# sevagh/demucs.cpp

Measured on AMD Instinct MI355X. Metric: audio-sec/s (xRT) htdemucs-4s 44.1kHz stereo, ~4-min track with overlap-add (BASELINE configs[2]), higher is better.
Workload: dtype f32 (exact bf16x3 operand split, fp32 accumulate)

## Files before the change

### demucs_cpp_amd/csrc/api.cpp

```cpp
#include "api_internal.h"
#include "tracks_plan.h"

#include <algorithm>
#include <atomic>
#include <cstdarg>
#include <cstdio>
#include <cstdlib>
#include <cmath>
#include <cstring>
#include <cctype>
#include <cerrno>
#include <climits>
#include <fcntl.h>
#include <pthread.h>
#include <signal.h>
#include <sys/mman.h>
#include <sys/stat.h>
#include <unistd.h>

using namespace dmx;

static thread_local std::string g_err;
int dmx_fail(int code, const char *fmt, ...)
{
// ... 2157 lines not shown
        rc = fail(DMX_ERR_HIP, "%s: hipMalloc failed", fn);
    if (rc == DMX_OK && (hipMemcpy(dIn, planes, inBytes, hipMemcpyHostToDevice) != hipSuccess ||
                         (mix && hipMemcpy(dMix, mix, mixBytes, hipMemcpyHostToDevice) != hipSuccess)))
        rc = fail(DMX_ERR_HIP, "%s: upload failed", fn);
    if (rc == DMX_OK)
        rc = dmx_remix_encode_device(device, dIn, n_sources, n, n, dMix, spec, dOut, dPeaks, nullptr);
    if (rc == DMX_OK && hipDeviceSynchronize() != hipSuccess)
        rc = fail(DMX_ERR_HIP, "%s: the kernels failed: %s", fn, hipGetErrorString(hipGetLastError()));
    for (int o = 0; rc == DMX_OK && o < nOut; ++o)
        if (hipMemcpy((unsigned char *)out + (size_t)(o * bytes), dOut + (size_t)(o * devStride), (size_t)bytes, hipMemcpyDeviceToHost) != hipSuccess)
            rc = fail(DMX_ERR_HIP, "%s: download failed", fn);
    if (rc == DMX_OK && peaks && hipMemcpy(peaks, dPeaks, sizeof(float) * (size_t)nOut, hipMemcpyDeviceToHost) != hipSuccess)
        rc = fail(DMX_ERR_HIP, "%s: download failed", fn);
    for (void *p : {(void *)dIn, (void *)dOut, (void *)dPeaks, (void *)dMix})
        if (p)
            (void)hipFree(p);
    return rc;
}

extern "C" int64_t dmx_flac_bound(int bits, int64_t n) { return flac_bound(bits, n); }
extern "C" int64_t dmx_flac_workspace_bytes(int bits, int64_t n) { return flac_workspace_bytes(bits, n); }

static int flac_check(const char *fn, int bits, int64_t n, int sample_rate)
{
    if (bits != 16 && bits != 24)
        return fail(DMX_ERR_ARG, "%s: bits %d (16 or 24)", fn, bits);
    if (n < 1 || n >= (int64_t)1 << 36)
        return fail(DMX_ERR_ARG, "%s: n = %lld, must be in [1, 2^36)", fn, (long long)n);
    if (sample_rate < 1 || sample_rate > 655350)
        return fail(DMX_ERR_ARG, "%s: sample_rate %d not in [1, 655350]", fn, sample_rate);
    return DMX_OK;
}

extern "C" int dmx_flac_encode_device(int device, const void *d_pcm, int bits, int64_t n, int sample_rate, void *d_out, int64_t *d_size,
                                      void *d_work, void *stream)
{
    const char *fn = "dmx_flac_encode_device";
    DMXCHK(flac_check(fn, bits, n, sample_rate));
    if (!d_pcm || !d_out || !d_size || !d_work)
        return fail(DMX_ERR_ARG, "%s: null %s pointer", fn, !d_pcm ? "d_pcm" : !d_out ? "d_out" : !d_size ? "d_size" : "d_work");
    if (((uintptr_t)d_pcm & 15) != 0 || ((uintptr_t)d_work & 15) != 0 || ((uintptr_t)d_size & 7) != 0)
        return fail(DMX_ERR_ARG, "%s: d_pcm and d_work must be 16-byte aligned, d_size 8-byte aligned", fn);
    HIPCHK(hipSetDevice(device));
    launch_flac_encode((const unsigned char *)d_pcm, 0, bits, n, sample_rate, 1, (unsigned char *)d_out, 0, (long long *)d_size,
                       (unsigned char *)d_work, (hipStream_t)stream);
    HIPCHK(hipGetLastError());
    return DMX_OK;
}

extern "C" int dmx_flac_encode(int device, const void *pcm, int bits, int64_t n, int sample_rate, void *out, int64_t *size)
{
    const char *fn = "dmx_flac_encode";
    DMXCHK(flac_check(fn, bits, n, sample_rate));
    if (!pcm || !out || !size)
        return fail(DMX_ERR_ARG, "%s: null %s pointer", fn, !pcm ? "pcm" : !out ? "out" : "size");
    HIPCHK(hipSetDevice(device));
    const size_t inBytes = (size_t)n * 2 * (size_t)(bits / 8);
    const i64 bound = flac_bound(bits, n), workBytes = flac_workspace_bytes(bits, n);
    unsigned char *dIn = nullptr, *dOut = nullptr, *dWork = nullptr;
    int64_t *dSize = nullptr;
    int64_t got = 0;
    int rc = DMX_OK;
    if (hipMalloc((void **)&dIn, DMX_OUTPUT_STRIDE(inBytes)) != hipSuccess || hipMalloc((void **)&dOut, (size_t)bound) != hipSuccess ||
        hipMalloc((void **)&dWork, (size_t)workBytes) != hipSuccess || hipMalloc((void **)&dSize, sizeof(int64_t)) != hipSuccess)
        rc = fail(DMX_ERR_HIP, "%s: hipMalloc failed", fn);
    if (rc == DMX_OK && hipMemcpy(dIn, pcm, inBytes, hipMemcpyHostToDevice) != hipSuccess)
        rc = fail(DMX_ERR_HIP, "%s: upload failed", fn);
    if (rc == DMX_OK)
        rc = dmx_flac_encode_device(device, dIn, bits, n, sample_rate, dOut, dSize, dWork, nullptr);
    if (rc == DMX_OK && hipDeviceSynchronize() != hipSuccess)
        rc = fail(DMX_ERR_HIP, "%s: the kernels failed: %s", fn, hipGetErrorString(hipGetLastError()));
    if (rc == DMX_OK && hipMemcpy(&got, dSize, sizeof(int64_t), hipMemcpyDeviceToHost) != hipSuccess)
        rc = fail(DMX_ERR_HIP, "%s: download failed", fn);
    if (rc == DMX_OK && (got < 42 || got > bound))
        rc = fail(DMX_ERR_HIP, "%s: internal error (%lld encoded bytes, bound %lld)", fn, (long long)got, (long long)bound);
    if (rc == DMX_OK && hipMemcpy(out, dOut, (size_t)got, hipMemcpyDeviceToHost) != hipSuccess)
        rc = fail(DMX_ERR_HIP, "%s: download failed", fn);
    for (void *p : {(void *)dIn, (void *)dOut, (void *)dWork, (void *)dSize})
        if (p)
            (void)hipFree(p);
    if (rc == DMX_OK)
        *size = got;
    return rc;
}

extern "C" int dmx_tracks_infer_flac(dmx_ctx *c, const dmx_model *const *models, int n_models, const float *weights, int n_tracks,
                                     const float *const *audio, const int64_t *n, int n_shifts, float overlap, const int *shift_offsets,
                                     const dmx_remix_spec *spec, int sample_rate, void *const *out, int64_t *sizes, float *peaks, int layout,
                                     dmx_progress_fn progress, void *user)
{
    TracksCall a = remix_call("dmx_tracks_infer_flac", c, models, n_models, weights, spec);
    a.kind = TRACKS_OUT_FLAC, a.flacRate = sample_rate, a.flacSizes = sizes;
    a.n_tracks = n_tracks, a.audio = audio, a.n = n, a.n_shifts = n_shifts, a.overlap = overlap, a.shift_offsets = shift_offsets;
    a.out = out, a.peaks = peaks, a.layout = layout, a.progress = progress, a.user = user;
    return tracks_call(a);
}

extern "C" int dmx_debug_tap(dmx_ctx *c, const char *name, int64_t *shape, float *host_dst)
{
    if (!c || !name || !shape || c->lastBatch < 1)
        return -1;
    (void)hipSetDevice(c->m->device);
    Plan *p = get_plan(c, c->lastBatch);
    for (const Op &op : p->ops)
        if (op.kind == OP_TAP && op.name == name)
        {
            int nd = 0;
            i64 per = 1;
            shape[nd++] = p->B;
            for (int j = 0; j < 4 && op.tap.shape[j] > 0; ++j)
            {
                shape[nd++] = op.tap.shape[j];
                per *= op.tap.shape[j];
            }
            if (host_dst)
            {
                (void)hipStreamSynchronize(c->stream);
                for (int b = 0; b < p->B; ++b)
                    if (hipMemcpy(host_dst + b * per, c->dA + op.tap.off + b * op.tap.batchStride, sizeof(float) * (size_t)per,
                                  hipMemcpyDeviceToHost) != hipSuccess)
                        return -1;
            }
            return nd;
        }
    return -1;
}

extern "C" int dmx_debug_n_ops(const dmx_ctx *c)
{
    if (!c)
        return 0;
    auto it = c->plans.find(c->maxBatch);
    return it == c->plans.end() ? 0 : (int)it->second->ops.size();
}

static void op_work(const Op &op, const char *&kernel, double &flops, double &bytes)
{
    static const char *cfgNames[] = {"igemm_128x128", "igemm_64x64", "igemm_128x96", "igemm_128x48", "igemm_256x16", "igemm_128x32",
                                     "igemm_128x64",  "igemm_64x128", "dgemm_direct", "igemm_64x64", "igemm_64x96", "igemm_64x48",
                                     "igemm_64x32",   "igemm_64x64",  "igemm_128x16", "igemm_32x128", "igemm_32x64", "igemm_256x128", "igemm_256x128w4", "igemm_lin256x128", "igemm_256x96"};
    static_assert(sizeof(cfgNames) / sizeof(cfgNames[0]) == kNumTileCfgs, "one label per tile configuration");
    flops = bytes = 0;
    kernel = "?";
    switch (op.kind)
    {
    case OP_IGEMM:
    {
        const IGemm &g = op.g;
        const double M = (double)g.B * g.P1 * g.P0;
        kernel = cfgNames[g.cfg];
        if (g.split)
        {
            static const char *splitNames[kNumTileCfgs] = {"igemm_split_128x128", nullptr, "igemm_split_128x96", "igemm_split_128x48", nullptr, "igemm_split_128x32d", "igemm_split_128x64d",
                                                            "igemm_split_64x128", nullptr, "igemm_split_64x64", "igemm_split_64x96", "igemm_split_64x48",
                                                            "igemm_split_128x32d", "igemm_split_128x64d", nullptr, "igemm_split_32x128", "igemm_split_32x64", nullptr, nullptr,
                                                            nullptr, nullptr};
            if (splitNames[g.cfg])
                kernel = splitNames[g.cfg];
            if (g.split == 2)
                kernel = g.cfg == 0 ? "igemm_splith_128x128" : g.cfg == 7 ? "igemm_splith_64x128" : kernel;
            else if (g.cfg == 0 || g.cfg == 2)
            {
                GemmArgs k{};
                fill_gemm_geometry(k, g);
                k.rowstat = g.rowstat >= 0 ? reinterpret_cast<float *>(1) : nullptr;
                const int wide = igemm_split_is_wide(g.cfg, k);
                if (wide)
                    kernel = wide == 256 ? "igemm_split_128x256" : wide == 192 ? "igemm_split_128x192" : "igemm_split_128x96d";
            }
        }
        flops = 2.0 * M * g.N * g.K;
        double in = (double)g.B * g.L1 * g.L0 * g.Cin, w = (double)g.N * g.K, out = 0;
        if (g.epi == EPI_LINEAR || g.epi == EPI_SCALE_RES)
            out = M * g.N;
        else if (g.epi == EPI_KPL || g.epi == EPI_VT)
            out = M * g.N;
        else if (g.epi == EPI_GLU || g.epi == EPI_GN_GLU_SCALE_RES)
            out = M * g.N / 2;
        else if (g.epi == EPI_TRCONV)
            out = (double)g.B * g.P1 * g.Lout * g.Cout;
        double res = g.res >= 0 ? out : 0;
        bytes = 4.0 * (in + w + out + res);
        break;
    }
    case OP_ATTENTION:
    {
        const Attention &t = op.at;
        kernel = t.split ? "attention_split" : "attention";
        flops = 4.0 * t.B * t.H * (double)t.Tq * t.Tk * t.hs;
        bytes = 4.0 * t.B * t.H * t.hs * (2.0 * t.Tq + 2.0 * t.Tk);
        break;
    }
    case OP_DCONV_ROW:
    {
        const DconvRow &r = op.dr;
        const double M = (double)r.B * r.T * r.F, hp = (r.hid + 3) / 4 * 4;
        kernel = "dconv_row";
        flops = 2.0 * (2.0 * M * hp * 3.0 * r.C + 2.0 * M * (hp + 2) * hp + 2.0 * M * 2.0 * r.C * hp);
        bytes = 4.0 * 2.0 * M * r.C;
        break;
    }
    case OP_STATS_REDUCE:
        kernel = "stats_reduce";
        bytes = 8.0 * op.sr.B * op.sr.R * op.sr.NB;
        break;
    case OP_STFT:
        kernel = "stft";
        flops = (double)op.stft.B * op.stft.T * 5.0 * 4096 * 12;
        bytes = 4.0 * op.stft.B * ((double)op.stft.seg * 2 + (double)op.stft.T * 2048 * 4);
        break;
    case OP_LAYERNORM:
        kernel = "layernorm";
        bytes = 8.0 * op.ln.rows * op.ln.D;
        break;
    case OP_GN_APPLY:
        kernel = "gn_apply";
        bytes = 8.0 * op.gn.B * op.gn.rows * op.gn.C;
        break;
    case OP_ISTFT:
        kernel = "istft";
        if (op.istft.fused)
            break;
        flops = (double)op.istft.B * op.istft.T * op.istft.S * 5.0 * 4096 * 12;
        bytes = 4.0 * op.istft.B * op.istft.T * op.istft.S * (2048.0 * 4 + 2 * 4096.0);
        break;
    case OP_OLA:
        kernel = "ola";
        bytes = 4.0 * op.ola.B * op.ola.S * 2 * ((double)op.ola.T * 4096 + 2.0 * op.ola.seg);
        if (op.ola.x >= 0)
        {
            kernel = "istft_ola";
            flops = (double)op.ola.B * op.ola.T * op.ola.S * 5.0 * 4096 * 12;
            bytes = 4.0 * op.ola.B * ((double)op.ola.T * 2048 * 4 * op.ola.S + 4.0 * op.ola.seg * op.ola.S);
        }
        break;
    case OP_GROUP_STATS:
        kernel = "group_stats";
        bytes = 4.0 * op.gs.B * op.gs.rows * op.gs.C;
        break;
    case OP_GN_ACT:
    {
        const GnAct &g = op.ga;
        const double Co = g.mode == 2 ? g.C / 2 : g.C;
        kernel = "gn_act";
        bytes = 4.0 * g.B * ((double)g.rowsOut * g.C + (double)g.rowsOut * Co * (g.res >= 0 ? 2 : 1));
        break;
    }
    case OP_LSTM:
    {
        const Lstm &l = op.lstm;
        kernel = "lstm";
        flops = 2.0 * l.B * l.T * 2.0 * 4.0 * l.H * l.H;
        bytes = 4.0 * (l.B * (double)l.T * 10.0 * l.H + 8.0 * l.H * l.H);
        break;
    }
    case OP_LOCAL_ATTN:
    {
        const LocalAttn &l = op.la;
        kernel = "local_attn";
        flops = 4.0 * l.B * (double)l.T * l.T * l.H;
        bytes = 4.0 * l.B * l.T * ((double)l.ld + l.H);
        break;
    }
    default:
        break;
    }
}

extern "C" int dmx_debug_profile(dmx_ctx *c, int batch, int reps, char *report, int report_cap)
{
    if (!c || batch < 1 || batch > c->maxBatch || reps < 1)
        return -1;
    (void)hipSetDevice(c->m->device);
    Plan *p = get_plan(c, batch);
    hipEvent_t e0, e1;
    if (hipEventCreate(&e0) != hipSuccess || hipEventCreate(&e1) != hipSuccess)
        return -1;
    int n = 0;
    std::string all;
    char line[512];
    for (const Op &op : p->ops)
    {
        if (op.kind == OP_TAP)
            continue;
        launch_op(c, op, c->stream, p->zeroOff);
        (void)hipEventRecord(e0, c->stream);
        for (int r = 0; r < reps; ++r)
            launch_op(c, op, c->stream, p->zeroOff);
        (void)hipEventRecord(e1, c->stream);
        (void)hipEventSynchronize(e1);
        float t = 0.f;
        (void)hipEventElapsedTime(&t, e0, e1);
        const char *kernel;
        double fl, by;
        op_work(op, kernel, fl, by);
        char geom[160] = "";
        if (op.kind == OP_IGEMM)
        {
            const IGemm &g = op.g;
            const i64 M = (i64)g.B * g.P1 * g.P0;
            const i64 tiles = ((M + kTileCfgs[g.cfg].BM - 1) / kTileCfgs[g.cfg].BM) * g.NB;
            snprintf(geom, sizeof(geom), "M=%lld N=%d K=%d tiles=%lld pro=%d epi=%d lin=%d stat=%d s%d", (long long)M, g.N, g.K, (long long)tiles,
                     g.pro, g.epi, (int)(g.S1 == 1 && g.pad0 == 0 && g.seg0 == g.K), (int)(g.rowstat >= 0), op.stream);
        }
        else
            snprintf(geom, sizeof(geom), "s%d", op.stream);
        snprintf(line, sizeof(line), "%s\t%s\t%.6f\t%.6e\t%.6e\t%s\n", op.name.c_str(), kernel, t / reps, fl, by, geom);
        all += line;
        ++n;
    }
    (void)hipEventDestroy(e0);
    (void)hipEventDestroy(e1);
    if (report && report_cap > 0)
    {
        size_t k = std::min((size_t)report_cap - 1, all.size());
        std::memcpy(report, all.data(), k);
        report[k] = 0;
    }
    return n;
}
```

### demucs_cpp_amd/csrc/dgemm.hip

```cpp
#include "kernels.h"
#include <cstdlib>

namespace dmx
{

typedef float f32x4 __attribute__((ext_vector_type(4)));

__device__ __forceinline__ float dgelu(float v) { return dmx_gelu(v); }
__device__ __forceinline__ float dsigmoid(float v) { return __builtin_amdgcn_rcpf(1.0f + __expf(-v)); }
__device__ __forceinline__ unsigned fdiv(unsigned n, const FastDiv f)
{
    return f.magic ? (__umulhi(n, f.magic) >> f.shift) : (n >> f.shift);
}
__device__ __forceinline__ float4 ld4z(const float *ptr, bool ok, const float *zero)
{
    const f32x4 v = *reinterpret_cast<const f32x4 *>(ok ? ptr : zero);
    return make_float4(v[0], v[1], v[2], v[3]);
}
__device__ __forceinline__ float f4get(const float4 &v, int c) { return c == 0 ? v.x : (c == 1 ? v.y : (c == 2 ? v.z : v.w)); }

template <int NF, int S1, int SEG0, int PRO, int EPI, int PIPE>
__global__ __launch_bounds__(256) void dgemm_kernel(const GemmArgs pa, const FastDiv dP0, const FastDiv dP1)
{
    GemmArgs p = pa;
    if (gridDim.y > 1)
    {
        const int n0 = (int)blockIdx.y * pa.N;
        p.Wt += (i64)n0 * pa.Kp, p.bias += n0, p.epiW += n0, p.epiB += n0, p.scale += n0 / 2;
        p.Y += n0 / 2, p.res += n0 / 2;
    }
    constexpr int NV4 = SEG0 / 16;
    constexpr int RPL = (SEG0 % 16) / 4;
    constexpr int NV4A = NV4 > 0 ? NV4 : 1;
    constexpr int RPLA = RPL > 0 ? RPL : 1;
    const int lane = threadIdx.x & 63, l15 = lane & 15, h = lane >> 4;
    const int gwave = blockIdx.x * 4 + (threadIdx.x >> 6), nwaves = gridDim.x * 4;
    const int rowLen = p.L0 * p.Cin;

    float4 Bv[NF][S1][NV4A];
    float Br[NF][S1][RPLA];
#pragma unroll
    for (int fj = 0; fj < NF; ++fj)
    {
        const int n = fj * 16 + l15;
        const float *w = p.Wt + (i64)(n < p.Np ? n : 0) * p.Kp;
        const bool nOk = n < p.Np;
#pragma unroll
        for (int s = 0; s < S1; ++s)
        {
#pragma unroll
            for (int j = 0; j < NV4; ++j)
                Bv[fj][s][j] = ld4z(w + s * SEG0 + 16 * j + 4 * h, nOk, p.zero);
#pragma unroll
            for (int c = 0; c < RPL; ++c)
                Br[fj][s][c] = nOk ? w[s * SEG0 + 16 * NV4 + RPL * h + c] : 0.f;
        }
    }
    float4 gW4[NV4A], gB4[NV4A];
    float gWr[RPLA], gBr[RPLA];
    if (PRO == PRO_GN_GELU)
    {
#pragma unroll
        for (int j = 0; j < NV4; ++j)
        {
            gW4[j] = *reinterpret_cast<const float4 *>(p.proW + 16 * j + 4 * h);
            gB4[j] = *reinterpret_cast<const float4 *>(p.proB + 16 * j + 4 * h);
        }
#pragma unroll
        for (int c = 0; c < RPL; ++c)
        {
            gWr[c] = p.proW[16 * NV4 + RPL * h + c];
            gBr[c] = p.proB[16 * NV4 + RPL * h + c];
        }
    }
    constexpr bool CST_LDS = EPI == EPI_GN_GLU_SCALE_RES;
    __shared__ float4 cst[CST_LDS ? 4 : 1][NF][4];
    float4 biasv[CST_LDS ? 1 : NF];
    int trR[NF], trC[NF];
    if (CST_LDS)
    {
        for (int i = threadIdx.x; i < NF * 4; i += 256)
        {
            const int fj = i >> 2, hh = i & 3, n = fj * 16 + 4 * hh;
            const bool ok = n < p.N;
            cst[0][fj][hh] = ld4z(p.bias + n, ok, p.zero);
            cst[CST_LDS ? 1 : 0][fj][hh] = ld4z(p.epiW + n, ok, p.zero);
            cst[CST_LDS ? 2 : 0][fj][hh] = ld4z(p.epiB + n, ok, p.zero);
            cst[CST_LDS ? 3 : 0][fj][hh] = ld4z(p.scale + (fj >> 1) * 16 + 4 * hh, ok && (fj & 1) == 0, p.zero);
        }
        __syncthreads();
    }
#pragma unroll
    for (int fj = 0; fj < NF; ++fj)
    {
        const int n = fj * 16 + 4 * h;
        if (!CST_LDS)
            biasv[fj] = ld4z(p.bias + n, n < p.N, p.zero);
        trR[fj] = trC[fj] = 0;
        if (EPI == EPI_TRCONV)
        {
            trR[fj] = n / p.Cout;
            trC[fj] = n - trR[fj] * p.Cout;
        }
    }

    constexpr int NRES = (EPI == EPI_GLU || EPI == EPI_GN_GLU_SCALE_RES) ? (NF + 1) / 2 : 1;
    struct Stage
    {
        unsigned m, b;
        int p0, p1;
        bool rowOk;
        float aMean, aScale, eMean, eSc;
        f32x4 a4[S1][NV4A];
        float ar[S1][RPLA];
        unsigned ok4, okr;
        f32x4 resv[NRES];
    };
    const int nfrag = (int)((p.M + 15) >> 4);
    const int C2 = p.N >> 1;
    auto fetch = [&](int frag, Stage &st) {
        const unsigned m = (unsigned)frag * 16u + (unsigned)l15;
        const bool rowOk = frag < nfrag && (i64)m < p.M;
        const unsigned mm = rowOk ? m : 0u;
        const unsigned t1 = fdiv(mm, dP0);
        const int p0 = (int)(mm - t1 * (unsigned)p.P0);
        const unsigned b = fdiv(t1, dP1);
        const int p1 = (int)(t1 - b * (unsigned)p.P1);
        const int grp = (int)b * p.G0 + (p.G0 > 1 ? p0 : 0);
        st.m = m, st.b = b, st.p0 = p0, st.p1 = p1, st.rowOk = rowOk;
        st.aMean = 0.f, st.aScale = 1.f, st.eMean = 0.f, st.eSc = 1.f;
        if (PRO == PRO_AFFINE)
        {
            st.aMean = p.proStats[b * 4];
            st.aScale = p.proStats[b * 4 + 1];
        }
        if (PRO == PRO_GN_GELU)
        {
            st.aMean = p.proStats[grp * 4];
            st.aScale = p.proStats[grp * 4 + 1];
        }
        if (EPI == EPI_GN_GLU_SCALE_RES)
        {
            st.eMean = p.epiStats[grp * 4];
            st.eSc = p.epiStats[grp * 4 + 1];
        }
        const int e0 = (p0 * p.stride0 - p.pad0) * p.Cin;
        const float *xb = p.X + (i64)b * p.xBS;
        st.ok4 = 0, st.okr = 0;
#pragma unroll
        for (int s = 0; s < S1; ++s)
        {
            const int in1 = p1 * p.stride1 + s * p.dil1 - p.pad1;
            const bool ok1 = rowOk && in1 >= 0 && in1 < p.L1;
            const float *rowp = xb + (i64)(ok1 ? in1 : 0) * rowLen;
#pragma unroll
            for (int j = 0; j < NV4; ++j)
            {
                const int e = e0 + 16 * j + 4 * h;
                const bool ok = ok1 && e >= 0 && e < rowLen;
                st.ok4 |= (ok ? 1u : 0u) << (s * NV4 + j);
                st.a4[s][j] = *reinterpret_cast<const f32x4 *>(ok ? rowp + e : p.zero);
            }
            if (RPL > 0)
            {
                const int e = e0 + 16 * NV4 + RPL * h;
                const bool ok = ok1 && e >= 0 && e < rowLen;
                st.okr |= (ok ? 1u : 0u) << s;
                const float *src = ok ? rowp + e : p.zero;
#pragma unroll
                for (int c = 0; c < RPL; ++c)
                    st.ar[s][c] = src[c];
            }
        }
#pragma unroll
        for (int r = 0; r < NRES; ++r)
            st.resv[r] = f32x4{0.f, 0.f, 0.f, 0.f};
        if (EPI == EPI_GLU || EPI == EPI_GN_GLU_SCALE_RES)
        {
#pragma unroll
            for (int r = 0; r < NRES; ++r)
            {
                const int c = r * 16 + 4 * h;
                if (rowOk && c < C2)
                {
                    if (EPI == EPI_GN_GLU_SCALE_RES)
                        st.resv[r] = *reinterpret_cast<const f32x4 *>(p.res + (i64)m * p.ldy + c);
                    else if (p.table)
                        st.resv[r] = *reinterpret_cast<const f32x4 *>(p.table + (i64)p0 * C2 + c);
                }
            }
        }
    };
    auto compute = [&](const Stage &st) {
        const float aMean = st.aMean, aScale = st.aScale;
        f32x4 acc[NF];
#pragma unroll
        for (int fj = 0; fj < NF; ++fj)
            acc[fj] = f32x4{0.f, 0.f, 0.f, 0.f};
#pragma unroll
        for (int s = 0; s < S1; ++s)
        {
#pragma unroll
            for (int j = 0; j < NV4; ++j)
            {
                f32x4 v = st.a4[s][j];
                if (PRO == PRO_AFFINE)
                {
                    v.x = (v.x - aMean) * aScale, v.y = (v.y - aMean) * aScale;
                    v.z = (v.z - aMean) * aScale, v.w = (v.w - aMean) * aScale;
                }
                if (PRO == PRO_GN_GELU)
                {
                    v.x = dgelu((v.x - aMean) * aScale * gW4[j].x + gB4[j].x);
                    v.y = dgelu((v.y - aMean) * aScale * gW4[j].y + gB4[j].y);
                    v.z = dgelu((v.z - aMean) * aScale * gW4[j].z + gB4[j].z);
                    v.w = dgelu((v.w - aMean) * aScale * gW4[j].w + gB4[j].w);
                }
                if (PRO != PRO_NONE && !((st.ok4 >> (s * NV4 + j)) & 1u))
                    v = f32x4{0.f, 0.f, 0.f, 0.f};
#pragma unroll
                for (int c = 0; c < 4; ++c)
#pragma unroll
                    for (int fj = 0; fj < NF; ++fj)
                        acc[fj] = __builtin_amdgcn_mfma_f32_16x16x4f32(f4get(Bv[fj][s][j], c), v[c], acc[fj], 0, 0, 0);
            }
#pragma unroll
            for (int c = 0; c < RPL; ++c)
            {
                float v = st.ar[s][c];
                if (PRO == PRO_AFFINE)
                    v = (v - aMean) * aScale;
                if (PRO == PRO_GN_GELU)
                    v = dgelu((v - aMean) * aScale * gWr[c] + gBr[c]);
                if (PRO != PRO_NONE && !((st.okr >> s) & 1u))
                    v = 0.f;
#pragma unroll
                for (int fj = 0; fj < NF; ++fj)
                    acc[fj] = __builtin_amdgcn_mfma_f32_16x16x4f32(Br[fj][s][c], v, acc[fj], 0, 0, 0);
            }
        }
        const i64 em = st.m;
        const bool eOk = st.rowOk;
        const int p0 = st.p0, p1 = st.p1;
        const unsigned b = st.b;
        float s = 0.f, ss = 0.f;
        if (EPI == EPI_LINEAR || EPI == EPI_STATS_ONLY || EPI == EPI_STATS_FACT)
        {
#pragma unroll
            for (int fj = 0; fj < NF; ++fj)
            {
                const int n = fj * 16 + 4 * h;
                if (eOk && n < p.N)
                {
                    const float4 bi = biasv[CST_LDS ? 0 : fj];
                    float4 v = make_float4(acc[fj][0] + bi.x, acc[fj][1] + bi.y, acc[fj][2] + bi.z, acc[fj][3] + bi.w);
                    if (EPI == EPI_LINEAR)
                    {
                        if (p.act)
                            v = make_float4(dgelu(v.x), dgelu(v.y), dgelu(v.z), dgelu(v.w));
                        *reinterpret_cast<float4 *>(p.Y + em * p.ldy + n) = v;
                    }
                    if (EPI == EPI_STATS_FACT)
                    {
                        const int hid = p.Cout;
                        const float vr[4] = {v.x, v.y, v.z, v.w};
#pragma unroll
                        for (int r = 0; r < 4; ++r)
                        {
                            const int nn = n + r;
                            ss += nn < hid ? vr[r] * vr[r] : (nn == hid + 1 ? 2.0f * vr[r] : 0.f);
                            s += nn == hid ? vr[r] : 0.f;
                        }
                    }
                    else
                    {
                        s += (v.x + v.y) + (v.z + v.w);
                        ss += (v.x * v.x + v.y * v.y) + (v.z * v.z + v.w * v.w);
                    }
                }
            }
            if (p.rowstat)
            {
                s += __shfl_xor(s, 16);
                ss += __shfl_xor(ss, 16);
                s += __shfl_xor(s, 32);
                ss += __shfl_xor(ss, 32);
                if (h == 0 && eOk)
                    *reinterpret_cast<float2 *>(p.rowstat + em * 2) = make_float2(s, ss);
            }
        }
        else if (EPI == EPI_GLU || EPI == EPI_GN_GLU_SCALE_RES)
        {
            if constexpr (NF % 2 == 0)
            {
                const float mean = st.eMean, sc = st.eSc;
#pragma unroll
                for (int fj = 0; fj < NF; fj += 2)
                {
                    const int c = (fj >> 1) * 16 + 4 * h;
                    if (eOk && c < C2)
                    {
                        const float4 ba = CST_LDS ? cst[0][fj][h] : biasv[CST_LDS ? 0 : fj];
                        const float4 bg = CST_LDS ? cst[0][fj + 1][h] : biasv[CST_LDS ? 0 : fj + 1];
                        float av[4] = {acc[fj][0] + ba.x, acc[fj][1] + ba.y, acc[fj][2] + ba.z, acc[fj][3] + ba.w};
                        float gv[4] = {acc[fj + 1][0] + bg.x, acc[fj + 1][1] + bg.y, acc[fj + 1][2] + bg.z, acc[fj + 1][3] + bg.w};
                        const f32x4 r4 = st.resv[fj >> 1];
                        const float rv[4] = {r4[0], r4[1], r4[2], r4[3]};
                        float ov[4];
                        if (EPI == EPI_GN_GLU_SCALE_RES)
                        {
                            const float4 gw4 = cst[CST_LDS ? 1 : 0][fj][h], gb4 = cst[CST_LDS ? 2 : 0][fj][h];
                            const float4 hw4 = cst[CST_LDS ? 1 : 0][fj + 1][h], hb4 = cst[CST_LDS ? 2 : 0][fj + 1][h];
                            const float4 sv4 = cst[CST_LDS ? 3 : 0][fj][h];
                            const float gw[4] = {gw4.x, gw4.y, gw4.z, gw4.w};
                            const float gb[4] = {gb4.x, gb4.y, gb4.z, gb4.w};
                            const float hw[4] = {hw4.x, hw4.y, hw4.z, hw4.w};
                            const float hb[4] = {hb4.x, hb4.y, hb4.z, hb4.w};
                            const float sv[4] = {sv4.x, sv4.y, sv4.z, sv4.w};
#pragma unroll
                            for (int r = 0; r < 4; ++r)
                            {
                                const float a = (av[r] - mean) * sc * gw[r] + gb[r];
                                const float g = (gv[r] - mean) * sc * hw[r] + hb[r];
                                ov[r] = rv[r] + sv[r] * (a * dsigmoid(g));
                            }
                        }
                        else
                        {
#pragma unroll
                            for (int r = 0; r < 4; ++r)
                                ov[r] = av[r] * dsigmoid(gv[r]) + p.tableScale * rv[r];
                        }
                        *reinterpret_cast<float4 *>(p.Y + em * p.ldy + c) = make_float4(ov[0], ov[1], ov[2], ov[3]);
                    }
                }
            }
        }
        else
        {
            i64 offs[NF];
#pragma unroll
            for (int fj = 0; fj < NF; ++fj)
            {
                const int n = fj * 16 + 4 * h;
                const int jj = p.trS * p0 + trR[fj] - p.trOff;
                offs[fj] = (eOk && n < p.N && jj >= 0 && jj < p.Lout) ? (i64)b * p.yBS + ((i64)p1 * p.Lout + jj) * p.ldy + trC[fj] : -1;
            }
#pragma unroll
            for (int fj = 0; fj < NF; ++fj)
                if (offs[fj] >= 0)
                {
                    const float4 bi = biasv[CST_LDS ? 0 : fj];
                    float4 v = make_float4(acc[fj][0] + bi.x, acc[fj][1] + bi.y, acc[fj][2] + bi.z, acc[fj][3] + bi.w);
                    if (p.act)
                        v = make_float4(dgelu(v.x), dgelu(v.y), dgelu(v.z), dgelu(v.w));
                    *reinterpret_cast<float4 *>(p.Y + offs[fj]) = v;
                }
        }
    };

    if constexpr (PIPE == 0)
    {
        Stage cur, nxt;
        fetch(gwave, cur);
        for (int frag = gwave; frag < nfrag; frag += nwaves)
        {
            fetch(frag + nwaves, nxt);
            compute(cur);
            cur = nxt;
        }
    }
    else if constexpr (PIPE == 3)
    {
        Stage s0, s1, s2;
        fetch(gwave, s0);
        fetch(gwave + nwaves, s1);
        for (int frag = gwave; frag < nfrag; frag += 3 * nwaves)
        {
            fetch(frag + 2 * nwaves, s2);
            compute(s0);
            fetch(frag + 3 * nwaves, s0);
            compute(s1);
            fetch(frag + 4 * nwaves, s1);
            compute(s2);
        }
    }
    else
    {
        Stage sa, sb;
        fetch(gwave, sa);
        for (int frag = gwave; frag < nfrag; frag += 2 * nwaves)
        {
            fetch(frag + nwaves, sb);
            if (PIPE == 2)
                __builtin_amdgcn_sched_barrier(0);
            compute(sa);
            if (PIPE == 2)
                __builtin_amdgcn_sched_barrier(0);
            fetch(frag + 2 * nwaves, sa);
            if (PIPE == 2)
                __builtin_amdgcn_sched_barrier(0);
            compute(sb);
            if (PIPE == 2)
                __builtin_amdgcn_sched_barrier(0);
        }
    }
}

template <int SEG0, int DIL, bool TIME>
__global__ __launch_bounds__(256) void dgemm_k1_ring_kernel(const GemmArgs p, const int len, const int nChunks, const int nFb)
{
    constexpr int NV4 = SEG0 / 16;
    constexpr int RING = 2 * DIL + 2;
    const int lane = threadIdx.x & 63, l15 = lane & 15, h = lane >> 4;
    const int gwave = blockIdx.x * 4 + (threadIdx.x >> 6), nwaves = gridDim.x * 4;
    const int T = p.P1, F = p.P0;
    const i64 rowLen = (i64)F * SEG0;

    f32x4 Bv[3][NV4];
    {
        const bool nOk = l15 < p.Np;
        const float *w = p.Wt + (i64)(nOk ? l15 : 0) * p.Kp;
#pragma unroll
        for (int s = 0; s < 3; ++s)
#pragma unroll
            for (int j = 0; j < NV4; ++j)
                Bv[s][j] = *reinterpret_cast<const f32x4 *>(nOk ? w + s * SEG0 + 16 * j + 4 * h : p.zero);
    }
    const int n = 4 * h;
    const float4 biasv = ld4z(p.bias + n, n < p.N, p.zero);

    const int ntask = p.B * nChunks * nFb;
    for (int task = gwave; task < ntask; task += nwaves)
    {
        const int fb = task % nFb, ck = (task / nFb) % nChunks, b = task / (nFb * nChunks);
        const int f = TIME ? 0 : fb * 16 + l15;
        const bool fOk = f < F;
        const int tl0 = TIME ? (ck * 16 + l15) * len : ck * len;
        const int tl1 = min(T, tl0 + len);
        const float *xb = p.X + (i64)b * p.xBS + (i64)(fOk ? f : 0) * SEG0 + 4 * h;
        f32x4 ring[RING][NV4];
        auto load_row = [&](int slot, int t) {
            const bool ok = fOk && t >= 0 && t < T && t < tl1 + DIL;
            const float *src = ok ? xb + (i64)t * rowLen : p.zero;
#pragma unroll
            for (int j = 0; j < NV4; ++j)
                ring[slot][j] = *reinterpret_cast<const f32x4 *>(ok ? src + 16 * j : src);
        };
#pragma unroll
        for (int i = 0; i <= 2 * DIL; ++i)
            load_row(i, tl0 - DIL + i);
        const int steps = TIME ? len : min(T, tl0 + len) - tl0;
        for (int ub = 0; ub < steps; ub += RING)
        {
#pragma unroll
            for (int u = 0; u < RING; ++u)
            {
                if (ub + u < steps)
                {
                    const int t = tl0 + ub + u;
                    load_row((u + 2 * DIL + 1) % RING, t + DIL + 1);
                    f32x4 acc = f32x4{0.f, 0.f, 0.f, 0.f};
#pragma unroll
                    for (int s = 0; s < 3; ++s)
#pragma unroll
                        for (int j = 0; j < NV4; ++j)
#pragma unroll
                            for (int c = 0; c < 4; ++c)
                                acc = __builtin_amdgcn_mfma_f32_16x16x4f32(Bv[s][j][c], ring[(u + s * DIL) % RING][j][c], acc, 0, 0, 0);
                    const bool rOk = fOk && t < tl1;
                    const i64 em = ((i64)b * T + t) * F + f;
                    float sm = 0.f, ss = 0.f;
                    if (rOk && n < p.N)
                    {
                        float4 v = make_float4(acc[0] + biasv.x, acc[1] + biasv.y, acc[2] + biasv.z, acc[3] + biasv.w);
                        if (p.act)
                            v = make_float4(dgelu(v.x), dgelu(v.y), dgelu(v.z), dgelu(v.w));
                        *reinterpret_cast<float4 *>(p.Y + em * p.ldy + n) = v;
                        sm += (v.x + v.y) + (v.z + v.w);
                        ss += (v.x * v.x + v.y * v.y) + (v.z * v.z + v.w * v.w);
                    }
                    if (p.rowstat)
                    {
                        sm += __shfl_xor(sm, 16);
                        ss += __shfl_xor(ss, 16);
                        sm += __shfl_xor(sm, 32);
                        ss += __shfl_xor(ss, 32);
                        if (h == 0 && rOk)
                            *reinterpret_cast<float2 *>(p.rowstat + em * 2) = make_float2(sm, ss);
                    }
                }
            }
        }
    }
}

template <int SEG0>
static void launch_k1_ring(const GemmArgs &a, hipStream_t s)
{
    const bool time = a.P0 == 1;
    const int nFb = time ? 1 : (a.P0 + 15) / 16;
    const i64 target = 4096;
    const i64 lanesRows = time ? (i64)a.B * a.P1 / 16 : (i64)a.B * nFb * a.P1;
    int len = (int)((lanesRows + target - 1) / target);
    len = len < 8 ? 8 : (len > 56 ? 56 : len);
    const int nChunks = time ? (a.P1 + 16 * len - 1) / (16 * len) : (a.P1 + len - 1) / len;
    const i64 ntask = (i64)a.B * nChunks * nFb;
    int blocks = (int)((ntask + 3) / 4);
    if (blocks > 256 * 8)
        blocks = 256 * 8;
#define DMX_K1(D, TM) hipLaunchKernelGGL((dgemm_k1_ring_kernel<SEG0, D, TM>), dim3(blocks), dim3(256), 0, s, a, len, nChunks, nFb)
    if (time && a.dil1 == 1)
        DMX_K1(1, true);
    else if (time)
        DMX_K1(2, true);
    else if (a.dil1 == 1)
        DMX_K1(1, false);
    else
        DMX_K1(2, false);
#undef DMX_K1
}
static bool k1_ring_ok(const GemmArgs &a)
{
    const char *e = getenv("DMX_K1_RING");
    const int on = e ? atoi(e) : 1;
    const bool timeOk = a.P0 == 1 && on != 2 && (on == 3 || (a.seg0 == 96 && (i64)a.B * a.P1 >= 12ll * 16 * 4096));
    return on && a.pro == PRO_NONE && a.epi == EPI_LINEAR && a.S1 == 3 && a.N <= 16 && (a.P0 >= 16 || timeOk) && a.L0 == a.P0 &&
           a.L1 == a.P1 && a.stride0 == 1 && a.stride1 == 1 && a.pad0 == 0 && a.pad1 == a.dil1 && (a.dil1 == 1 || a.dil1 == 2) &&
           a.seg0 == a.Cin && a.NB == 1 && !a.res;
}

template <int NF, int S1, int SEG0, int PRO, int EPI, int PIPE_>
static void launch_d(const GemmArgs &a, hipStream_t s, int chunks = 1)
{
    const int nfrag = (int)((a.M + 15) >> 4);
    int blocks = (nfrag + 3) / 4;
    if (blocks > 256 * 8 / chunks)
        blocks = 256 * 8 / chunks;
    constexpr int PIPE = PIPE_;
    hipLaunchKernelGGL((dgemm_kernel<NF, S1, SEG0, PRO, EPI, PIPE>), dim3(blocks, chunks), dim3(256), 0, s, a, make_fastdiv((unsigned)a.P0),
                       make_fastdiv((unsigned)a.P1));
}

int launch_dgemm(const GemmArgs &a, hipStream_t s, bool dry)
{
    const int NF = (a.N + 15) / 16;
    if (a.M >= (1ll << 31) - 16 || (i64)a.L0 * a.Cin >= (1ll << 31))
        return -1;
    if ((a.epi == EPI_LINEAR || a.epi == EPI_TRCONV) && a.res)
        return -1;
#define DMX_D(NF_, S1_, SEG_, PRO_, EPI_, PIPE_)                              \
    case (NF_ * 1000000 + S1_ * 100000 + SEG_ * 100 + PRO_ * 10 + EPI_):      \
        if (!dry)                                                             \
            launch_d<NF_, S1_, SEG_, PRO_, EPI_, PIPE_>(a, s);                \
        return 0;
    if (k1_ring_ok(a) && (a.seg0 == 48 || a.seg0 == 96))
    {
        if (!dry)
            a.seg0 == 48 ? launch_k1_ring<48>(a, s) : launch_k1_ring<96>(a, s);
        return 0;
    }
    if (a.pro == PRO_GN_GELU && a.epi == EPI_GN_GLU_SCALE_RES && a.S1 == 1 && (a.seg0 == 24 || a.seg0 == 48) && a.N > 192 && a.N % 192 == 0)
    {
        if (!dry)
        {
            const int cw = 96;
            GemmArgs c = a;
            c.N = c.Np = cw;
            const int chunks = a.N / cw;
            if (cw == 192)
                a.seg0 == 24 ? launch_d<12, 1, 24, PRO_GN_GELU, EPI_GN_GLU_SCALE_RES, 1>(c, s, chunks) : launch_d<12, 1, 48, PRO_GN_GELU, EPI_GN_GLU_SCALE_RES, 0>(c, s, chunks);
            else
                a.seg0 == 24 ? launch_d<6, 1, 24, PRO_GN_GELU, EPI_GN_GLU_SCALE_RES, 0>(c, s, chunks) : launch_d<6, 1, 48, PRO_GN_GELU, EPI_GN_GLU_SCALE_RES, 0>(c, s, chunks);
        }
        return 0;
    }
    switch (NF * 1000000 + a.S1 * 100000 + a.seg0 * 100 + a.pro * 10 + a.epi)
    {
        DMX_D(1, 3, 48, PRO_NONE, EPI_LINEAR, 0)
        DMX_D(1, 3, 96, PRO_NONE, EPI_LINEAR, 1)
        DMX_D(6, 1, 8, PRO_GN_GELU, EPI_STATS_ONLY, 2)
        DMX_D(1, 1, 8, PRO_GN_GELU, EPI_STATS_FACT, 0)
        DMX_D(1, 1, 12, PRO_GN_GELU, EPI_STATS_FACT, 0)
        DMX_D(6, 1, 8, PRO_GN_GELU, EPI_GN_GLU_SCALE_RES, 0)
        DMX_D(12, 1, 12, PRO_GN_GELU, EPI_STATS_ONLY, 0)
        DMX_D(12, 1, 12, PRO_GN_GELU, EPI_GN_GLU_SCALE_RES, 1)
        DMX_D(6, 1, 12, PRO_GN_GELU, EPI_GN_GLU_SCALE_RES, 0)
        DMX_D(12, 1, 24, PRO_GN_GELU, EPI_GN_GLU_SCALE_RES, 1)
        DMX_D(2, 1, 24, PRO_GN_GELU, EPI_STATS_FACT, 0)
        DMX_D(3, 1, 32, PRO_AFFINE, EPI_LINEAR, 0)
        DMX_D(3, 1, 16, PRO_AFFINE, EPI_LINEAR, 0)
        DMX_D(6, 1, 48, PRO_NONE, EPI_GLU, 0)
        DMX_D(4, 1, 96, PRO_NONE, EPI_TRCONV, 0)
        DMX_D(2, 1, 96, PRO_NONE, EPI_TRCONV, 0)
        DMX_D(6, 1, 96, PRO_NONE, EPI_TRCONV, 0)
        DMX_D(3, 1, 96, PRO_NONE, EPI_TRCONV, 0)
    default:
        return -1;
    }
#undef DMX_D
}

}
```

### demucs_cpp_amd/csrc/kernels.h

```cpp
#pragma once
#include "plan.h"
#include <hip/hip_runtime.h>
#include <cstdlib>

namespace dmx
{

struct FastDiv
{
    unsigned magic, shift;
};
inline FastDiv make_fastdiv(unsigned d)
{
    FastDiv f;
    f.magic = 0;
    f.shift = 0;
    if (d == 0)
        d = 1;
    if ((d & (d - 1)) == 0)
    {
        while ((1u << f.shift) < d)
            ++f.shift;
        return f;
    }
    unsigned s = 0;
    while ((1ull << s) < d)
        ++s;
    f.magic = (unsigned)((((unsigned long long)1 << (31 + s)) + d - 1) / d);
    f.shift = s - 1;
    return f;
}

struct GemmArgs
{
    const float *X;
    i64 xBS;
    int B, P1, P0, L1, L0, Cin;
    int S1, stride1, dil1, pad1, seg0, stride0, pad0, K, Kp;
    int pro;
    const float *proStats, *proW, *proB;
    int G0;
    const float *Wt, *bias;
    const unsigned short *Wb1, *Wb2;
    int N, Np;
    int epi, act;
    float *Y;
    i64 yBS;
    int ldy;
    const float *res, *scale, *epiStats, *epiW, *epiB;
    float *rowstat;
    int NB;
    const float *table;
    float tableScale;
    int Lout, Cout;
    int trS, trOff;
    const float *rowScale;
    unsigned short *kvPl;
    i64 kvPlane;
    int kvCol0, kvT, kvH, kvHs;
    i64 M;
    const float *zero;
    unsigned tilesM, tilesN;
    FastDiv dP0, dP1;
    int xcdMap;
};

int launch_dgemm(const GemmArgs &a, hipStream_t s, bool dry = false);

struct DconvRowArgs
{
    float *x;
    int B, T, F, C, hid;
    const float *img[2];
    float eps;
    const float *zero;
    int rowsPerXcd;
    double n1, invN1, invN1m1, n2, invN2, invN2m1;
};
int launch_dconv_row(const DconvRowArgs &a, hipStream_t s, bool dry = false);

int launch_igemm(int cfg, const GemmArgs &a, hipStream_t s, bool dry = false);
int launch_igemm_lin256(const GemmArgs &a, hipStream_t s, bool dry = false);
int launch_igemm_split(int cfg, const GemmArgs &a, hipStream_t s, bool dry = false, int arith = 0);
int igemm_split_is_wide(int cfg, const GemmArgs &a);
void launch_rowscale(const GemmArgs &a, float *out, hipStream_t s);
void launch_split3h_debug(const float *d_x, i64 n, int sexp, unsigned short *d_planes, hipStream_t s);
void launch_split3_debug(const float *d_x, i64 n, unsigned short *d_planes, hipStream_t s);

struct ReduceArgs
{
    const float *rowstat;
    float *out;
    int B, R, NB, G0;
    double count;
    int mode;
    float eps;
    double *scratch;
    int nchunk;
};
void launch_stats_reduce(const ReduceArgs &a, hipStream_t s);

struct StftArgs
{
    const float *mix;
    float *x, *rowstat, *rowstatT;
    int B, T, seg, pad;
    const float *window, *twiddle;
};
void launch_stft(const StftArgs &a, hipStream_t s);

struct LnArgs
{
    const float *x;
    float *y;
    int rows, D, rowsPerBatch;
    const float *w, *b, *pe;
    float eps;
};
void launch_layernorm(const LnArgs &a, hipStream_t s);

struct GnArgs
{
    const float *x;
    float *y;
    const float *res;
    int B, rows, C;
    const float *stats, *w, *b;
};
void launch_gn_apply(const GnArgs &a, hipStream_t s);

struct AttnArgs
{
    const float *q, *k, *v;
    float *o;
    int ldq, ldk, ldv, ldo;
    i64 qB, kB, vB, oB;
    int B, Tq, Tk, H, hs;
    float scale;
    unsigned nQt;
    int xcdMap;
    const float *decay;
    int ldd;
    i64 dB;
    const unsigned short *kpl, *vt;
    i64 kvPlane;
};

void launch_attention(const AttnArgs &a, hipStream_t s);
int launch_attention_split(const AttnArgs &a, hipStream_t s, bool dry = false);
int launch_attention_local(const AttnArgs &a, hipStream_t s);

struct IstftArgs
{
    const float *x, *stats;
    float *frames;
    int B, T, S;
    const float *window, *twiddle;
};
void launch_istft(const IstftArgs &a, hipStream_t s);

struct OlaArgs
{
    const float *frames, *xt, *statsT, *wss;
    float *out;
    int B, T, S, seg, pad;
};
void launch_ola(const OlaArgs &a, hipStream_t s);
struct IstftOlaArgs
{
    const float *x, *stats, *xt, *statsT, *wss, *window, *twiddle;
    float *out;
    int B, T, S, seg, pad;
    int nch, fpc;
    const float *rden;
};
void launch_istft_ola(const IstftOlaArgs &a, hipStream_t s);

struct GroupStatsArgs
{
    const float *x;
    float *out;
    double *partials;
    int B, rows, C, G;
    float eps;
};
void launch_group_stats(const GroupStatsArgs &a, hipStream_t s);
struct GnActArgs
{
    const float *x;
    float *y;
    const float *stats, *res, *w, *b, *scale;
    int B, rowsIn, C, G, mode, rowOff, rowsOut;
};
void launch_gn_act(const GnActArgs &a, hipStream_t s);
struct LstmArgs
{
    const float *xproj, *whh;
    float *out;
    void *gran;
    unsigned *status;
    int B, T, H;
};
int launch_lstm(const LstmArgs &a, hipStream_t s);
struct LocalAttnArgs
{
    const float *qkvd;
    float *out;
    int B, T, H, ld;
};
int launch_local_attn(const LocalAttnArgs &a, hipStream_t s);

struct TrackStatsTable
{
    static const int kMax = 32;
    const float *audio[kMax];
    i64 n[kMax];
    float *stats[kMax];
};
void launch_track_stats(const TrackStatsTable &t, int T, double *partials, int nblk, hipStream_t s);
void launch_track_stats_final(const TrackStatsTable &t, int T, const double *partials, int nblk, hipStream_t s);
void launch_track_stats(const float *audio, i64 n, double *partials, int nblk, hipStream_t s);
void launch_track_stats_final(const double *partials, int nblk, i64 n, float *stats, hipStream_t s);
struct TrackSegItem
{
    const float *audio;
    const float *stats;
    i64 n;
    int shift;
    int seg;
};
struct TrackSegIdx
{
    static const int kMax = 64;
    TrackSegItem v[kMax];
};
void launch_track_gather(const TrackSegItem *items, int nIdx, i64 seg, i64 stride, float *mixes, hipStream_t s);
void launch_track_gather(const float *audio, i64 n, const float *stats, int shiftOffset, i64 seg, i64 stride,
                         i64 len, const int *segIdx, int nIdx, float *mixes, hipStream_t s);
struct TrackOlaEntry
{
    const float *segOut;
    const float *stats;
    float *out;
    i64 n, len, i0, i1;
    i64 gBase, slot0;
    int nSeg, shift;
};
struct TrackOlaTable
{
    static const int kMax = 32;
    TrackOlaEntry e[kMax];
};
void launch_track_ola(const TrackOlaEntry *entries, int T, int S, i64 seg, i64 stride, i64 ring, int layout, int planeBase,
                      int nPlanes, hipStream_t s);
void launch_track_ola(const float *segOut, int nSeg, int S, i64 seg, i64 stride, i64 len, i64 n, int shiftOffset,
                      const float *stats, float *out, int layout, int planeBase, int nPlanes, i64 i0, i64 i1, hipStream_t s,
                      int gBase = 0);
struct TrackEnsPiece
{
    const float *stats;
    float *out;
    i64 n, i0, i1;
    i64 itemLo, slotLo;
    int nMin, nTail;
};
struct TrackEnsCopy
{
    int shift, nseg;
};
struct TrackEnsTable
{
    static const int kMaxPieces = 16, kMaxCopies = 256;
    static const int kMaxTail = 2048;
    TrackEnsPiece p[kMaxPieces];
    TrackEnsCopy c[kMaxCopies];
};
void launch_track_ola_ens(const TrackEnsPiece *pieces, const TrackEnsCopy *copies, int P, int N, const float *segOut, int S,
                          i64 seg, i64 stride, i64 ring, int layout, int planeBase, int nPlanes, hipStream_t s);
struct TrackBagPiece
{
    const float *stats;
    float *out;
    i64 n, i0, i1;
};
struct TrackBagModel
{
    int itemLo, slotLo;
    int nMin, nTail;
};
struct TrackBagTable
{
    static const int kMaxPieces = 8, kMaxModels = 32, kMaxCopies = 256, kMaxBag = 8, kMaxStems = 8;
    static const int kMaxTail = 12288;
    TrackBagPiece p[kMaxPieces];
    TrackBagModel m[kMaxModels];
    TrackEnsCopy c[kMaxCopies];
    float w[kMaxBag * kMaxStems];
    const float *ring[kMaxBag];
    i64 ringBlocks[kMaxBag];
};
i64 track_ola_bag_tail_entries(const TrackBagModel *models, int P, int Q, int N, int S, const float *w);
bool launch_track_ola_bag(const TrackBagPiece *pieces, const TrackBagModel *models, const TrackEnsCopy *copies, int P, int Q, int N,
                          const float *w, const float *const *rings, const i64 *ringBlocks, int S, i64 seg, i64 stride, int layout,
                          int planeBase, int nPlanes, hipStream_t s);
struct PcmPiece
{
    const float *planes;
    unsigned char *pcm;
    unsigned *peaks;
    i64 n, planeStride, outStride, i0, i1;
};
struct PcmTable
{
    static const int kMax = 32;
    PcmPiece p[kMax];
};
void launch_pcm_peak(const PcmPiece *pieces, int P, int S, int stem, hipStream_t s);
void launch_pcm_encode(const PcmPiece *pieces, int P, int S, int stem, int encoding, int clip, hipStream_t s);
struct PcmGains
{
    static const int kMaxOut = 8, kMaxSrc = 7;
    float g[kMaxOut][kMaxSrc];
    int nOut, S;
};
struct RemixPiece : PcmPiece
{
    const float *mix;
};
struct RemixTable
{
    static const int kMax = 32;
    RemixPiece p[kMax];
};
void launch_remix_peak(const RemixPiece *pieces, int P, const PcmGains &G, hipStream_t s);
void launch_remix_encode(const RemixPiece *pieces, int P, const PcmGains &G, int encoding, int clip, hipStream_t s);
i64 flac_bound(int bits, i64 n);
i64 flac_workspace_bytes(int bits, i64 n);
void launch_flac_encode(const unsigned char *pcm, i64 pcmStride, int bits, i64 n, int rate, int nOut, unsigned char *out, i64 outStride,
                        long long *sizes, unsigned char *work, hipStream_t s);
void launch_copy_rows(float *dst, i64 dpitch, const float *src, i64 spitch, i64 width, int rows, hipStream_t s);
void launch_f32_to_f16(const float *src, unsigned short *dst, i64 n, hipStream_t s);
void launch_planar_to_interleaved(const float *src, float *dst, i64 n, hipStream_t s);


#ifdef __HIPCC__
__device__ __forceinline__ float dmx_erff(float x)
{
    const float t = fminf(fabsf(x), 4.0f);
    const float s = x * x;
    float a = fmaf(-0.0005843715625815094f, s, 0.004958246368914843f);
    a = fmaf(a, s, -0.026736384257674217f);
    a = fmaf(a, s, 0.11280667781829834f);
    a = fmaf(a, s, -0.3761231601238251f);
    a = fmaf(a, s, 1.1283791065216064f);
    a *= x;
    float b = fmaf(0.0002812488819472492f, t, -0.004376694560050964f);
    b = fmaf(b, t, 0.03201308846473694f);
    b = fmaf(b, t, -0.149833083152771f);
    b = fmaf(b, t, -0.9193801283836365f);
    b = fmaf(b, t, -1.6268224716186523f);
    b = fmaf(b, t, -0.0002986486360896379f);
    const float r = copysignf(1.0f - __builtin_amdgcn_exp2f(b), x);
    return t < 0.92f ? a : r;
}
__device__ __forceinline__ float dmx_gelu(float v) { return 0.5f * v * (1.0f + dmx_erff(v * 0.70710678118654752440f)); }
#endif

}
```

Before: 3101.

## Add per-wave LDS-staged slab kernel for small-N K=3 time convolutions

Adds a new direct-conv kernel for the 3-tap time-axis convolutions with N<=16 (DConv layers). Each wave stages a slab of input rows, including the halo, into its own LDS region and reuses them across the three taps. It prefetches the next slab into registers while computing the current one with fp32 MFMA, and fuses bias, GELU and rowstat. It replaces the ring kernel or generic path for these shapes by default, aiming to cut redundant global loads and improve latency hiding. The cost is extra LDS use and halo reloads per slab, and the slab size is picked by a heuristic.

```diff
diff --git a/demucs_cpp_amd/csrc/api.cpp b/demucs_cpp_amd/csrc/api.cpp
--- a/demucs_cpp_amd/csrc/api.cpp
+++ b/demucs_cpp_amd/csrc/api.cpp
@@ -2483,6 +2483,14 @@
             const i64 tiles = ((M + kTileCfgs[g.cfg].BM - 1) / kTileCfgs[g.cfg].BM) * g.NB;
             snprintf(geom, sizeof(geom), "M=%lld N=%d K=%d tiles=%lld pro=%d epi=%d lin=%d stat=%d s%d", (long long)M, g.N, g.K, (long long)tiles,
                      g.pro, g.epi, (int)(g.S1 == 1 && g.pad0 == 0 && g.seg0 == g.K), (int)(g.rowstat >= 0), op.stream);
+            if (g.cfg == kDirectCfg)
+            {
+                GemmArgs k{};
+                fill_gemm_geometry(k, g);
+                k.res = g.res >= 0 ? reinterpret_cast<const float *>(1) : nullptr;
+                const size_t n0 = strlen(geom);
+                snprintf(geom + n0, sizeof(geom) - n0, " stg=%d", dgemm_k1_staged_slab(k));
+            }
         }
         else
             snprintf(geom, sizeof(geom), "s%d", op.stream);
diff --git a/demucs_cpp_amd/csrc/dgemm.hip b/demucs_cpp_amd/csrc/dgemm.hip
--- a/demucs_cpp_amd/csrc/dgemm.hip
+++ b/demucs_cpp_amd/csrc/dgemm.hip
@@ -1,4 +1,5 @@
 #include "kernels.h"
+#include "dgemm_slab.h"
 #include <cstdlib>
 
 namespace dmx
@@ -530,6 +531,129 @@
            a.seg0 == a.Cin && a.NB == 1 && !a.res;
 }
 
+template <int SEG0, int DIL, int SLAB>
+__global__ __launch_bounds__(256, SEG0 == 48 ? 4 : SLAB == 16 ? 3 : 2) void dgemm_k1_staged_kernel(const GemmArgs p)
+{
+    constexpr int NV4 = SEG0 / 16, C4 = SEG0 / 4;
+    constexpr int ROWS = SLAB + 2 * DIL, PITCH = SEG0 + 8;
+    constexpr int NLD = (ROWS * C4 + 63) / 64;
+    __shared__ float regions[4][ROWS * PITCH];
+    const int lane = threadIdx.x & 63, l15 = lane & 15, h = lane >> 4;
+    float *const slab = regions[threadIdx.x >> 6];
+    const int gwave = blockIdx.x * 4 + (threadIdx.x >> 6), nwaves = gridDim.x * 4;
+    const int L = p.P1;
+
+    f32x4 Bv[3][NV4];
+    {
+        const bool nOk = l15 < p.Np;
+        const float *w = p.Wt + (i64)(nOk ? l15 : 0) * p.Kp;
+#pragma unroll
+        for (int s = 0; s < 3; ++s)
+#pragma unroll
+            for (int j = 0; j < NV4; ++j)
+                Bv[s][j] = *reinterpret_cast<const f32x4 *>(nOk ? w + s * SEG0 + 16 * j + 4 * h : p.zero);
+    }
+    const int n = 4 * h;
+    const float4 biasv = ld4z(p.bias + n, n < p.N, p.zero);
+
+    const int ntask = p.B * k1_slabs_per_segment(L, SLAB);
+    f32x4 st[NLD];
+    auto load_slab = [&](int task) {
+        const K1Slab s = k1_slab(task < ntask ? task : 0, L, SLAB);
+        const i64 base = (i64)s.b * p.xBS + ((i64)s.t0 - DIL) * SEG0;
+#pragma unroll
+        for (int it = 0; it < NLD; ++it)
+        {
+            const int i = it * 64 + lane, r = i / C4;
+            const bool ok = task < ntask && r < ROWS && k1_slab_row_time(s, r, DIL, L) >= 0;
+            st[it] = *reinterpret_cast<const f32x4 *>(ok ? p.X + (base + 4 * i) : p.zero);
+        }
+    };
+    load_slab(gwave);
+    for (int task = gwave; task < ntask; task += nwaves)
+    {
+        const K1Slab s = k1_slab(task, L, SLAB);
+#pragma unroll
+        for (int it = 0; it < NLD; ++it)
+        {
+            const int i = it * 64 + lane, r = i / C4;
+            if (r < ROWS)
+                *reinterpret_cast<f32x4 *>(slab + r * PITCH + 4 * (i - r * C4)) = st[it];
+        }
+        __builtin_amdgcn_fence(__ATOMIC_RELEASE, "wavefront");
+        __builtin_amdgcn_wave_barrier();
+        __builtin_amdgcn_fence(__ATOMIC_ACQUIRE, "wavefront");
+        load_slab(task + nwaves);
+#pragma unroll
+        for (int f = 0; f < SLAB / 16; ++f)
+        {
+            if (16 * f < s.nOut)
+            {
+                f32x4 acc = f32x4{0.f, 0.f, 0.f, 0.f};
+#pragma unroll
+                for (int tap = 0; tap < 3; ++tap)
+#pragma unroll
+                    for (int j = 0; j < NV4; ++j)
+                    {
+                        const f32x4 v = *reinterpret_cast<const f32x4 *>(slab + (16 * f + l15 + tap * DIL) * PITCH + 16 * j + 4 * h);
+#pragma unroll
+                        for (int c = 0; c < 4; ++c)
+                            acc = __builtin_amdgcn_mfma_f32_16x16x4f32(Bv[tap][j][c], v[c], acc, 0, 0, 0);
+                    }
+                const int t = s.t0 + 16 * f + l15;
+                const bool rOk = t < L;
+                const i64 em = (i64)s.b * L + t;
+                float sm = 0.f, ss = 0.f;
+                if (rOk && n < p.N)
+                {
+                    float4 v = make_float4(acc[0] + biasv.x, acc[1] + biasv.y, acc[2] + biasv.z, acc[3] + biasv.w);
+                    if (p.act)
+                        v = make_float4(dgelu(v.x), dgelu(v.y), dgelu(v.z), dgelu(v.w));
+                    *reinterpret_cast<float4 *>(p.Y + em * p.ldy + n) = v;
+                    sm += (v.x + v.y) + (v.z + v.w);
+                    ss += (v.x * v.x + v.y * v.y) + (v.z * v.z + v.w * v.w);
+                }
+                if (p.rowstat)
+                {
+                    sm += __shfl_xor(sm, 16);
+                    ss += __shfl_xor(ss, 16);
+                    sm += __shfl_xor(sm, 32);
+                    ss += __shfl_xor(ss, 32);
+                    if (h == 0 && rOk)
+                        *reinterpret_cast<float2 *>(p.rowstat + em * 2) = make_float2(sm, ss);
+                }
+            }
+        }
+        __builtin_amdgcn_fence(__ATOMIC_RELEASE, "wavefront");
+        __builtin_amdgcn_wave_barrier();
+    }
+}
+
+int dgemm_k1_staged_slab(const GemmArgs &a)
+{
+    const char *e = getenv("DMX_K1_STAGED");
+    const int on = e ? atoi(e) : 1;
+    const bool shape = a.P0 == 1 && a.pro == PRO_NONE && a.epi == EPI_LINEAR && a.S1 == 3 && a.N <= 16 && a.L0 == 1 && a.L1 == a.P1 &&
+                       a.stride0 == 1 && a.stride1 == 1 && a.pad0 == 0 && a.pad1 == a.dil1 && (a.dil1 == 1 || a.dil1 == 2) &&
+                       a.seg0 == a.Cin && (a.seg0 == 48 || a.seg0 == 96) && a.NB == 1 && !a.res && a.M < (1ll << 31) - 64;
+    if (on <= 0 || !shape)
+        return 0;
+    return a.seg0 == 96 && (on == 3 || (i64)a.B * a.P1 >= 16ll * 4 * 256 * 12) ? 16 : 32;
+}
+
+template <int SEG0, int SLAB>
+static void launch_k1_staged(const GemmArgs &a, hipStream_t s)
+{
+    const i64 ntask = (i64)a.B * k1_slabs_per_segment(a.P1, SLAB);
+    int blocks = (int)((ntask + 3) / 4);
+    if (blocks > 256 * 8)
+        blocks = 256 * 8;
+    if (a.dil1 == 1)
+        hipLaunchKernelGGL((dgemm_k1_staged_kernel<SEG0, 1, SLAB>), dim3(blocks), dim3(256), 0, s, a);
+    else
+        hipLaunchKernelGGL((dgemm_k1_staged_kernel<SEG0, 2, SLAB>), dim3(blocks), dim3(256), 0, s, a);
+}
+
 template <int NF, int S1, int SEG0, int PRO, int EPI, int PIPE_>
 static void launch_d(const GemmArgs &a, hipStream_t s, int chunks = 1)
 {
@@ -554,6 +678,12 @@
         if (!dry)                                                             \
             launch_d<NF_, S1_, SEG_, PRO_, EPI_, PIPE_>(a, s);                \
         return 0;
+    if (const int slab = dgemm_k1_staged_slab(a))
+    {
+        if (!dry)
+            a.seg0 == 48 ? launch_k1_staged<48, 32>(a, s) : slab == 16 ? launch_k1_staged<96, 16>(a, s) : launch_k1_staged<96, 32>(a, s);
+        return 0;
+    }
     if (k1_ring_ok(a) && (a.seg0 == 48 || a.seg0 == 96))
     {
         if (!dry)
diff --git a/demucs_cpp_amd/csrc/dgemm_slab.h b/demucs_cpp_amd/csrc/dgemm_slab.h
--- /dev/null
+++ b/demucs_cpp_amd/csrc/dgemm_slab.h
@@ -0,0 +1,37 @@
+#pragma once
+
+#if defined(__HIPCC__)
+#define DMX_SLAB_HD __host__ __device__
+#else
+#define DMX_SLAB_HD
+#endif
+
+namespace dmx
+{
+
+struct K1Slab
+{
+    int b;
+    int t0;
+    int nOut;
+};
+
+DMX_SLAB_HD inline int k1_slabs_per_segment(int L, int slab) { return (L + slab - 1) / slab; }
+
+DMX_SLAB_HD inline K1Slab k1_slab(int task, int L, int slab)
+{
+    const int per = k1_slabs_per_segment(L, slab);
+    K1Slab s;
+    s.b = task / per;
+    s.t0 = (task - s.b * per) * slab;
+    s.nOut = L - s.t0 < slab ? L - s.t0 : slab;
+    return s;
+}
+
+DMX_SLAB_HD inline int k1_slab_row_time(const K1Slab &s, int r, int d, int L)
+{
+    const int t = s.t0 - d + r;
+    return (t >= 0 && t < L) ? t : -1;
+}
+
+}
diff --git a/demucs_cpp_amd/csrc/kernels.h b/demucs_cpp_amd/csrc/kernels.h
--- a/demucs_cpp_amd/csrc/kernels.h
+++ b/demucs_cpp_amd/csrc/kernels.h
@@ -66,6 +66,7 @@
 };
 
 int launch_dgemm(const GemmArgs &a, hipStream_t s, bool dry = false);
+int dgemm_k1_staged_slab(const GemmArgs &a);
 
 struct DconvRowArgs
 {
```

New measurement: 3113, median of 6. About the same (+0.4%).
